# chacorp/latent-nerf-test

Measured on AMD Instinct MI355X. Metric: latent-frames/sec (64x64x4, 128^3 grid), render forward+backward, higher is better.
Workload: dtype bf16

## Files before the change

### latent-nerf-test_amd/csrc/grid_gather.hip

```cpp
#include "grid_shared.h"

namespace lnerf {

template <typename TT> struct CellRaw;
template <> struct CellRaw<uint16_t> {
    uint32_t d[8];
    __device__ __forceinline__ void load_pair(const uint16_t *lt, uint32_t row, int c) {
        const uint2 v = *reinterpret_cast<const uint2 *>(lt + (int64_t)row * 2);
        d[c] = v.x; d[c + 1] = v.y;
    }
    __device__ __forceinline__ void load_one(const uint16_t *lt, uint32_t row, int c) {
        d[c] = reinterpret_cast<const uint32_t *>(lt)[row];
    }
    __device__ __forceinline__ void load_quad(const uint16_t *lt, uint32_t r0, uint32_t r1, int c) {
        const uint4 v = *reinterpret_cast<const uint4 *>(lt + (int64_t)(r0 & ~3u) * 2);
        const uint32_t k0 = r0 & 3u, k1 = r1 & 3u;
        d[c] = (k0 & 2u) ? ((k0 & 1u) ? v.w : v.z) : ((k0 & 1u) ? v.y : v.x);
        d[c + 1] = (k1 & 2u) ? ((k1 & 1u) ? v.w : v.z) : ((k1 & 1u) ? v.y : v.x);
    }
    static constexpr bool kHasQuad = true;
    __device__ __forceinline__ void swap_pair(int c) { const uint32_t t = d[c]; d[c] = d[c + 1]; d[c + 1] = t; }
    __device__ __forceinline__ void zero() {
#pragma unroll
        for (int i = 0; i < 8; ++i) d[i] = 0u;
    }
    __device__ __forceinline__ void take_from_lane(int src) {
#pragma unroll
        for (int i = 0; i < 8; ++i) d[i] = (uint32_t)__builtin_amdgcn_ds_bpermute(src << 2, (int)d[i]);
    }
    __device__ __forceinline__ float2 get(int c) const {
        return make_float2(__uint_as_float(d[c] << 16), __uint_as_float(d[c] & 0xFFFF0000u));
    }
};
template <> struct CellRaw<float> {
    float2 d[8];
    __device__ __forceinline__ void load_pair(const float *lt, uint32_t row, int c) {
        const float4 v = *reinterpret_cast<const float4 *>(lt + (int64_t)row * 2);
        d[c] = make_float2(v.x, v.y); d[c + 1] = make_float2(v.z, v.w);
    }
    __device__ __forceinline__ void load_one(const float *lt, uint32_t row, int c) {
        d[c] = reinterpret_cast<const float2 *>(lt)[row];
    }
    __device__ __forceinline__ void load_quad(const float *, uint32_t, uint32_t, int) {}
    static constexpr bool kHasQuad = false;
    __device__ __forceinline__ void swap_pair(int c) { const float2 t = d[c]; d[c] = d[c + 1]; d[c + 1] = t; }
    __device__ __forceinline__ void zero() {
#pragma unroll
        for (int i = 0; i < 8; ++i) d[i] = make_float2(0.f, 0.f);
    }
    __device__ __forceinline__ void take_from_lane(int src) {
#pragma unroll
        for (int i = 0; i < 8; ++i) {
            d[i].x = __int_as_float(__builtin_amdgcn_ds_bpermute(src << 2, __float_as_int(d[i].x)));
            d[i].y = __int_as_float(__builtin_amdgcn_ds_bpermute(src << 2, __float_as_int(d[i].y)));
        }
    }
    __device__ __forceinline__ float2 get(int c) const { return d[c]; }
};

template <typename TT, typename TO>
__global__ void __launch_bounds__(256)
k_grid_forward(const float *__restrict__ xyzs, float bound, const TT *__restrict__ table, GridMeta meta, int64_t m_host,
               const int32_t *__restrict__ m_dev, int64_t level_stride, TO *__restrict__ feat, int pair_loads,
               int dedup_max_res) {
    int64_t M = m_host;
    if (m_dev) { const int64_t md = *m_dev; M = md < M ? md : M; }
    const TileMap tm = tile_map(0, meta.num_levels);
    const int l = tm.level;
    const float scale = meta.scales[l];
    const uint32_t res = (uint32_t)meta.res[l];
    const uint32_t off = (uint32_t)meta.offsets[l];
    const uint32_t hsize = (uint32_t)(meta.offsets[l + 1] - meta.offsets[l]);
    const TT *lt = table + (int64_t)off * 2;
    const bool dense = (uint64_t)(res + 1) * (res + 1) * (res + 1) <= (uint64_t)hsize;
    const bool pow2 = (hsize & (hsize - 1u)) == 0u;
    const bool dedup = (int)res <= dedup_max_res;
    const int lane = lane_id();
    for (int64_t tile = tm.tile0; tile * 256 < M; tile += tm.tstep) {
        const int64_t m = tile * 256 + threadIdx.x;
        const bool valid = m < M;
        LevelPos p;
        p.gx = p.gy = p.gz = 0u; p.fx = p.fy = p.fz = 0.f;
        if (valid) p = level_pos(xyzs, m, bound, scale);
        uint32_t rows[8];
        corner_rows(p.gx, p.gy, p.gz, res, hsize, rows, meta.blocked);
        bool fetch = valid;
        int src = lane;
        if (dedup) {
            const RunInfo ri = wave_cell_runs(p.gx, p.gy, p.gz, valid, lane);
            src = ri.start;
            fetch = valid && ri.start == lane;
        }
        CellRaw<TT> cell;
        cell.zero();
        if (fetch) {
            if (pair_loads && dense) {
#pragma unroll
                for (int c = 0; c < 8; c += 2) cell.load_pair(lt, rows[c], c);
            } else if (meta.blocked == 2) {
#pragma unroll
                for (int c = 0; c < 8; ++c) cell.load_one(lt, rows[c], c);
            } else if (pair_loads == 2 && CellRaw<TT>::kHasQuad && pow2 && (p.gx & 3u) != 3u) {
#pragma unroll
                for (int c = 0; c < 8; c += 2) cell.load_quad(lt, rows[c], rows[c + 1], c);
            } else if (pair_loads && pow2 && !(p.gx & 1u)) {
#pragma unroll
                for (int c = 0; c < 8; c += 2) {
                    cell.load_pair(lt, rows[c] & ~1u, c);
                    if (rows[c] & 1u) cell.swap_pair(c);
                }
            } else {
#pragma unroll
                for (int c = 0; c < 8; ++c) cell.load_one(lt, rows[c], c);
            }
        }
        if (dedup) cell.take_from_lane(src);
        float a0 = 0.f, a1 = 0.f;
#pragma unroll
        for (int c = 0; c < 8; ++c) {
            const uint32_t bx = c & 1, by = (c >> 1) & 1, bz = (c >> 2) & 1;
            const float wx = bx ? p.fx : 1.0f - p.fx;
            const float wy = by ? p.fy : 1.0f - p.fy;
            const float wz = bz ? p.fz : 1.0f - p.fz;
            const float w = (wx * wy) * wz;
            const float2 v = cell.get(c);
            a0 = fmaf(w, v.x, a0);
            a1 = fmaf(w, v.y, a1);
        }
        if (valid) Feat2<TO>::store(feat, (int64_t)l * level_stride + m, a0, a1);
    }
}

template <typename TG>
__global__ void __launch_bounds__(256)
k_grid_backward_atomic(const float *__restrict__ xyzs, float bound, const TG *__restrict__ dfeat, GridMeta meta,
                       int64_t m_host, const int32_t *__restrict__ m_dev, int64_t level_stride,
                       float *__restrict__ dtable, int variant) {
    int64_t M = m_host;
    if (m_dev) { const int64_t md = *m_dev; M = md < M ? md : M; }
    const TileMap tm = tile_map(variant, meta.num_levels);
    if (!tm.ok) return;
    const int l = tm.level;
    const float scale = meta.scales[l];
    const uint32_t res = (uint32_t)meta.res[l];
    const uint32_t off = (uint32_t)meta.offsets[l];
    const uint32_t hsize = (uint32_t)(meta.offsets[l + 1] - meta.offsets[l]);
    float *lt = dtable + (int64_t)off * 2;
    for (int64_t tile = tm.tile0; tile * 256 < M; tile += tm.tstep) {
        const int64_t m = tile * 256 + threadIdx.x;
        if (m >= M) continue;
        const LevelPos p = level_pos(xyzs, m, bound, scale);
        const float2 gg = Feat2<TG>::load(dfeat + ((int64_t)l * level_stride + m) * 2, 0);
        uint32_t rows[8];
        corner_rows(p.gx, p.gy, p.gz, res, hsize, rows, meta.blocked);
#pragma unroll
        for (int c = 0; c < 8; ++c) {
            const uint32_t bx = c & 1, by = (c >> 1) & 1, bz = (c >> 2) & 1;
            const uint32_t row = rows[c];
            const float wx = bx ? p.fx : 1.0f - p.fx;
            const float wy = by ? p.fy : 1.0f - p.fy;
            const float wz = bz ? p.fz : 1.0f - p.fz;
            const float w = (wx * wy) * wz;
            atomicAdd(lt + (int64_t)row * 2, w * gg.x);
            atomicAdd(lt + (int64_t)row * 2 + 1, w * gg.y);
        }
    }
}

static void launch_dims(int variant, int L, int64_t m_host, dim3 &grid) {
    const int64_t tiles = div_up(m_host, 256);
    if (variant == 0) {
        int64_t gx = tiles < 1 ? 1 : tiles;
        if (gx > 2048) gx = 2048;
        grid = dim3((unsigned)gx, (unsigned)L, 1);
    } else {
        const int lv_per_xcd = (L + 7) / 8;
        int64_t per_level = tiles < 1 ? 1 : tiles;
        if (per_level > 256) per_level = 256;
        grid = dim3((unsigned)(8 * lv_per_xcd * per_level), 1, 1);
    }
}

void launch_grid_backward_atomic(const float *xyzs, float bound, const float *dfeat, const GridMeta &meta, int64_t m_host,
                                 const int32_t *m_dev, int64_t level_stride, float *dtable, int variant, hipStream_t s) {
    dim3 grid;
    launch_dims(variant, meta.num_levels, m_host, grid);
    hipLaunchKernelGGL((k_grid_backward_atomic<float>), grid, dim3(256), 0, s, xyzs, bound, dfeat, meta, m_host, m_dev,
                       level_stride, dtable, variant);
}

}

using namespace lnerf;

extern "C" {

int lnerf_grid_encode_forward(const float *xyzs, float bound, const void *table, int table_dtype, int num_levels,
                              int level_dim, const int32_t *offsets_host, const float *scales_host,
                              const int32_t *res_host, int64_t m_host, const int32_t *m_dev, int64_t level_stride,
                              void *feat, int feat_dtype, int variant, lnerf_stream_t stream) {
    GridMeta meta;
    const int blocked = variant & (LNERF_GRID_BLOCKED | LNERF_GRID_TILED);
    variant &= ~(LNERF_GRID_BLOCKED | LNERF_GRID_TILED);
    int rc = fill_meta("grid_encode_forward", meta, num_levels, level_dim, offsets_host, scales_host, res_host, blocked);
    if (rc) return rc;
    LNERF_REQUIRE(m_host >= 0 && level_stride >= m_host, "grid_encode_forward: need 0 <= m_host <= level_stride");
    LNERF_REQUIRE(bound > 0.f, "grid_encode_forward: bound must be > 0");
    LNERF_REQUIRE(variant == 0, "grid_encode_forward: unknown variant %d", variant);
    LNERF_REQUIRE((table_dtype == LNERF_F32 || table_dtype == LNERF_BF16) &&
                      (feat_dtype == LNERF_F32 || feat_dtype == LNERF_BF16),
                  "grid_encode_forward: bad dtype tag");
    if (m_host == 0) return LNERF_OK;
    LNERF_REQUIRE(xyzs && table && feat, "grid_encode_forward: null pointer");
    dim3 grid;
    launch_dims(0, num_levels, m_host, grid);
    hipStream_t s = as_stream(stream);
#define LAUNCH_FWD(TT, TO)                                                                                         \
    hipLaunchKernelGGL((k_grid_forward<TT, TO>), grid, dim3(256), (size_t)g_gather_lds_pad, s, xyzs, bound, (const TT *)table, meta, m_host, \
                       m_dev, level_stride, (TO *)feat, g_gather_pairs, g_gather_dedup_res)
    if (table_dtype == LNERF_F32 && feat_dtype == LNERF_F32) LAUNCH_FWD(float, float);
    else if (table_dtype == LNERF_F32) LAUNCH_FWD(float, uint16_t);
    else if (feat_dtype == LNERF_F32) LAUNCH_FWD(uint16_t, float);
    else LAUNCH_FWD(uint16_t, uint16_t);
#undef LAUNCH_FWD
    LNERF_CHECK_LAUNCH("grid_encode_forward");
    return LNERF_OK;
}

}
```

Measured before the change: 2751.

## Specialize grid forward gather by span and prefetch next tile positions

Turns the runtime choice of gather path (dense pair, quad, pair, single loads) into template specializations, so each kernel instance carries one straight-line load path. The position of the next tile is loaded ahead of time, with sched barriers and asm register pins to overlap that load with the current gather. Row addresses are computed with 32-bit offsets, and a host check rejects levels larger than 4 GiB. The pins and prefetch add register pressure and can cut occupancy. The feature pointer offset now multiplies by 2, which may change indexing if Feat2 store already accounted for two channels.

```diff
diff --git a/latent-nerf-test_amd/csrc/grid_gather.hip b/latent-nerf-test_amd/csrc/grid_gather.hip
--- a/latent-nerf-test_amd/csrc/grid_gather.hip
+++ b/latent-nerf-test_amd/csrc/grid_gather.hip
@@ -1,28 +1,49 @@
 #include "grid_shared.h"
 
 namespace lnerf {
+
+typedef uint32_t u32x2 __attribute__((ext_vector_type(2)));
+typedef uint32_t u32x4 __attribute__((ext_vector_type(4)));
+
+template <typename TT> __device__ __forceinline__ const uint32_t *row_ptr(const TT *lt, uint32_t row) {
+    return reinterpret_cast<const uint32_t *>(reinterpret_cast<const char *>(lt) + (size_t)(row * (uint32_t)(2 * sizeof(TT))));
+}
 
 template <typename TT> struct CellRaw;
 template <> struct CellRaw<uint16_t> {
+    u32x4 a[4];
     uint32_t d[8];
-    __device__ __forceinline__ void load_pair(const uint16_t *lt, uint32_t row, int c) {
-        const uint2 v = *reinterpret_cast<const uint2 *>(lt + (int64_t)row * 2);
-        d[c] = v.x; d[c + 1] = v.y;
-    }
-    __device__ __forceinline__ void load_one(const uint16_t *lt, uint32_t row, int c) {
-        d[c] = reinterpret_cast<const uint32_t *>(lt)[row];
-    }
-    __device__ __forceinline__ void load_quad(const uint16_t *lt, uint32_t r0, uint32_t r1, int c) {
-        const uint4 v = *reinterpret_cast<const uint4 *>(lt + (int64_t)(r0 & ~3u) * 2);
-        const uint32_t k0 = r0 & 3u, k1 = r1 & 3u;
-        d[c] = (k0 & 2u) ? ((k0 & 1u) ? v.w : v.z) : ((k0 & 1u) ? v.y : v.x);
-        d[c + 1] = (k1 & 2u) ? ((k1 & 1u) ? v.w : v.z) : ((k1 & 1u) ? v.y : v.x);
-    }
-    static constexpr bool kHasQuad = true;
-    __device__ __forceinline__ void swap_pair(int c) { const uint32_t t = d[c]; d[c] = d[c + 1]; d[c + 1] = t; }
-    __device__ __forceinline__ void zero() {
-#pragma unroll
-        for (int i = 0; i < 8; ++i) d[i] = 0u;
+    static constexpr int kMaxSpan = 4;
+    static constexpr int kOwn = 8;
+    template <int SPAN> __device__ __forceinline__ void load_a(const uint16_t *lt, uint32_t row, int i) {
+        const uint32_t *p = row_ptr(lt, row);
+        if (SPAN == 4) {
+            a[i] = *reinterpret_cast<const u32x4 *>(p);
+        } else {
+            const u32x2 v = *reinterpret_cast<const u32x2 *>(p);
+            a[i].x = v.x; a[i].y = v.y;
+        }
+    }
+    __device__ __forceinline__ void load_own(const uint16_t *lt, uint32_t row, int c) { d[c] = *row_ptr(lt, row); }
+    __device__ __forceinline__ void open_raw() {
+        asm volatile("" : "=v"(a[0]), "=v"(a[1]), "=v"(a[2]), "=v"(a[3]), "=v"(d[0]), "=v"(d[1]), "=v"(d[2]), "=v"(d[3]),
+                          "=v"(d[4]), "=v"(d[5]), "=v"(d[6]), "=v"(d[7]));
+    }
+    __device__ __forceinline__ void pin_raw() {
+        asm volatile("" : "+v"(a[0]), "+v"(a[1]), "+v"(a[2]), "+v"(a[3]), "+v"(d[0]), "+v"(d[1]), "+v"(d[2]), "+v"(d[3]),
+                          "+v"(d[4]), "+v"(d[5]), "+v"(d[6]), "+v"(d[7]));
+    }
+    template <int SPAN> static __device__ __forceinline__ uint32_t pick(const u32x4 &v, uint32_t k) {
+        if (SPAN == 2) return (k & 1u) ? v.y : v.x;
+        return (k & 2u) ? ((k & 1u) ? v.w : v.z) : ((k & 1u) ? v.y : v.x);
+    }
+    template <int SPAN, bool DENSE> __device__ __forceinline__ void take_pairs(const uint32_t rows[8], bool own) {
+        if (SPAN == 1 || own) return;
+#pragma unroll
+        for (int i = 0; i < 4; ++i) {
+            d[2 * i] = DENSE ? a[i].x : pick<SPAN>(a[i], rows[2 * i]);
+            d[2 * i + 1] = DENSE ? a[i].y : pick<SPAN>(a[i], rows[2 * i + 1]);
+        }
     }
     __device__ __forceinline__ void take_from_lane(int src) {
 #pragma unroll
@@ -33,57 +54,75 @@
     }
 };
 template <> struct CellRaw<float> {
-    float2 d[8];
-    __device__ __forceinline__ void load_pair(const float *lt, uint32_t row, int c) {
-        const float4 v = *reinterpret_cast<const float4 *>(lt + (int64_t)row * 2);
-        d[c] = make_float2(v.x, v.y); d[c + 1] = make_float2(v.z, v.w);
-    }
-    __device__ __forceinline__ void load_one(const float *lt, uint32_t row, int c) {
-        d[c] = reinterpret_cast<const float2 *>(lt)[row];
-    }
-    __device__ __forceinline__ void load_quad(const float *, uint32_t, uint32_t, int) {}
-    static constexpr bool kHasQuad = false;
-    __device__ __forceinline__ void swap_pair(int c) { const float2 t = d[c]; d[c] = d[c + 1]; d[c + 1] = t; }
-    __device__ __forceinline__ void zero() {
-#pragma unroll
-        for (int i = 0; i < 8; ++i) d[i] = make_float2(0.f, 0.f);
+    u32x4 a[4];
+    u32x2 d[8];
+    static constexpr int kMaxSpan = 2;
+    static constexpr int kOwn = 4;
+    template <int SPAN> __device__ __forceinline__ void load_a(const float *lt, uint32_t row, int i) {
+        const uint32_t *p = row_ptr(lt, row);
+        if (SPAN == 2) {
+            a[i] = *reinterpret_cast<const u32x4 *>(p);
+        } else {
+            const u32x2 v = *reinterpret_cast<const u32x2 *>(p);
+            a[i].x = v.x; a[i].y = v.y;
+        }
+    }
+    __device__ __forceinline__ void load_own(const float *lt, uint32_t row, int c) {
+        d[c] = *reinterpret_cast<const u32x2 *>(row_ptr(lt, row));
+    }
+    __device__ __forceinline__ void open_raw() {
+        asm volatile("" : "=v"(a[0]), "=v"(a[1]), "=v"(a[2]), "=v"(a[3]), "=v"(d[1]), "=v"(d[3]), "=v"(d[5]), "=v"(d[7]));
+    }
+    __device__ __forceinline__ void pin_raw() {
+        asm volatile("" : "+v"(a[0]), "+v"(a[1]), "+v"(a[2]), "+v"(a[3]), "+v"(d[1]), "+v"(d[3]), "+v"(d[5]), "+v"(d[7]));
+    }
+    static __device__ __forceinline__ u32x2 pick(const u32x4 &v, uint32_t k) {
+        return (k & 1u) ? u32x2{v.z, v.w} : u32x2{v.x, v.y};
+    }
+    template <int SPAN, bool DENSE> __device__ __forceinline__ void take_pairs(const uint32_t rows[8], bool own) {
+#pragma unroll
+        for (int i = 0; i < 4; ++i) d[2 * i] = (SPAN == 1 || DENSE) ? u32x2{a[i].x, a[i].y} : pick(a[i], rows[2 * i]);
+        if (SPAN == 1 || own) return;
+#pragma unroll
+        for (int i = 0; i < 4; ++i) d[2 * i + 1] = DENSE ? u32x2{a[i].z, a[i].w} : pick(a[i], rows[2 * i + 1]);
     }
     __device__ __forceinline__ void take_from_lane(int src) {
 #pragma unroll
         for (int i = 0; i < 8; ++i) {
-            d[i].x = __int_as_float(__builtin_amdgcn_ds_bpermute(src << 2, __float_as_int(d[i].x)));
-            d[i].y = __int_as_float(__builtin_amdgcn_ds_bpermute(src << 2, __float_as_int(d[i].y)));
-        }
-    }
-    __device__ __forceinline__ float2 get(int c) const { return d[c]; }
+            d[i].x = (uint32_t)__builtin_amdgcn_ds_bpermute(src << 2, (int)d[i].x);
+            d[i].y = (uint32_t)__builtin_amdgcn_ds_bpermute(src << 2, (int)d[i].y);
+        }
+    }
+    __device__ __forceinline__ float2 get(int c) const { return make_float2(__uint_as_float(d[c].x), __uint_as_float(d[c].y)); }
 };
 
-template <typename TT, typename TO>
-__global__ void __launch_bounds__(256)
-k_grid_forward(const float *__restrict__ xyzs, float bound, const TT *__restrict__ table, GridMeta meta, int64_t m_host,
-               const int32_t *__restrict__ m_dev, int64_t level_stride, TO *__restrict__ feat, int pair_loads,
-               int dedup_max_res) {
-    int64_t M = m_host;
-    if (m_dev) { const int64_t md = *m_dev; M = md < M ? md : M; }
-    const TileMap tm = tile_map(0, meta.num_levels);
-    const int l = tm.level;
-    const float scale = meta.scales[l];
-    const uint32_t res = (uint32_t)meta.res[l];
-    const uint32_t off = (uint32_t)meta.offsets[l];
-    const uint32_t hsize = (uint32_t)(meta.offsets[l + 1] - meta.offsets[l]);
-    const TT *lt = table + (int64_t)off * 2;
-    const bool dense = (uint64_t)(res + 1) * (res + 1) * (res + 1) <= (uint64_t)hsize;
-    const bool pow2 = (hsize & (hsize - 1u)) == 0u;
-    const bool dedup = (int)res <= dedup_max_res;
+struct PosRaw {
+    float x, y, z;
+    __device__ __forceinline__ void request(const float *__restrict__ xyzs, int64_t m, int64_t M) {
+        m = m < M ? m : M - 1;
+        x = xyzs[m * 3]; y = xyzs[m * 3 + 1]; z = xyzs[m * 3 + 2];
+    }
+    __device__ __forceinline__ void pin() { asm volatile("" : "+v"(x), "+v"(y), "+v"(z)); }
+};
+
+template <typename TT, typename TO, int SPAN, bool DENSE>
+__device__ __forceinline__ void gather_tiles(const float *__restrict__ xyzs, float bound, const TT *__restrict__ lt,
+                                             float scale, uint32_t res, uint32_t hsize, int layout, bool dedup, int64_t M,
+                                             const TileMap &tm, TO *__restrict__ lfeat) {
+    constexpr uint32_t kmask = DENSE ? 0u : (uint32_t)(SPAN - 1);
     const int lane = lane_id();
+    PosRaw pos;
+    pos.request(xyzs, tm.tile0 * 256 + threadIdx.x, M);
+    pos.pin();
     for (int64_t tile = tm.tile0; tile * 256 < M; tile += tm.tstep) {
         const int64_t m = tile * 256 + threadIdx.x;
         const bool valid = m < M;
-        LevelPos p;
-        p.gx = p.gy = p.gz = 0u; p.fx = p.fy = p.fz = 0.f;
-        if (valid) p = level_pos(xyzs, m, bound, scale);
+        PosRaw next;
+        next.request(xyzs, m + tm.tstep * 256 < M ? m + tm.tstep * 256 : m, M);
+        __builtin_amdgcn_sched_barrier(0);
+        const LevelPos p = level_pos_xyz(pos.x, pos.y, pos.z, bound, scale);
         uint32_t rows[8];
-        corner_rows(p.gx, p.gy, p.gz, res, hsize, rows, meta.blocked);
+        corner_rows(p.gx, p.gy, p.gz, res, hsize, rows, layout);
         bool fetch = valid;
         int src = lane;
         if (dedup) {
@@ -91,29 +130,21 @@
             src = ri.start;
             fetch = valid && ri.start == lane;
         }
+        const bool own = SPAN == 1 || (!DENSE && (p.gx & (uint32_t)(SPAN - 1)) == (uint32_t)(SPAN - 1));
         CellRaw<TT> cell;
-        cell.zero();
+        cell.open_raw();
         if (fetch) {
-            if (pair_loads && dense) {
-#pragma unroll
-                for (int c = 0; c < 8; c += 2) cell.load_pair(lt, rows[c], c);
-            } else if (meta.blocked == 2) {
-#pragma unroll
-                for (int c = 0; c < 8; ++c) cell.load_one(lt, rows[c], c);
-            } else if (pair_loads == 2 && CellRaw<TT>::kHasQuad && pow2 && (p.gx & 3u) != 3u) {
-#pragma unroll
-                for (int c = 0; c < 8; c += 2) cell.load_quad(lt, rows[c], rows[c + 1], c);
-            } else if (pair_loads && pow2 && !(p.gx & 1u)) {
-#pragma unroll
-                for (int c = 0; c < 8; c += 2) {
-                    cell.load_pair(lt, rows[c] & ~1u, c);
-                    if (rows[c] & 1u) cell.swap_pair(c);
-                }
-            } else {
-#pragma unroll
-                for (int c = 0; c < 8; ++c) cell.load_one(lt, rows[c], c);
+            if (CellRaw<TT>::kOwn == 4 || (SPAN > 1 && !own)) {
+#pragma unroll
+                for (int i = 0; i < 4; ++i) cell.template load_a<SPAN>(lt, rows[2 * i] & ~kmask, i);
             }
-        }
+            if (own) {
+#pragma unroll
+                for (int c = (CellRaw<TT>::kOwn == 4 ? 1 : 0); c < 8; c += 8 / CellRaw<TT>::kOwn) cell.load_own(lt, rows[c], c);
+            }
+        }
+        cell.pin_raw();
+        cell.template take_pairs<SPAN, DENSE>(rows, own);
         if (dedup) cell.take_from_lane(src);
         float a0 = 0.f, a1 = 0.f;
 #pragma unroll
@@ -127,8 +158,45 @@
             a0 = fmaf(w, v.x, a0);
             a1 = fmaf(w, v.y, a1);
         }
-        if (valid) Feat2<TO>::store(feat, (int64_t)l * level_stride + m, a0, a1);
-    }
+        next.pin();
+        if (valid) Feat2<TO>::store(lfeat, m, a0, a1);
+        pos = next;
+    }
+}
+
+template <typename TT, typename TO>
+__global__ void __launch_bounds__(256)
+k_grid_forward(const float *__restrict__ xyzs, float bound, const TT *__restrict__ table, GridMeta meta, int64_t m_host,
+               const int32_t *__restrict__ m_dev, int64_t level_stride, TO *__restrict__ feat, int pair_loads,
+               int dedup_max_res) {
+    int64_t M = m_host;
+    if (m_dev) { const int64_t md = *m_dev; M = md < M ? md : M; }
+    const TileMap tm = tile_map(0, meta.num_levels);
+    if (tm.tile0 * 256 >= M) return;
+    const int l = tm.level;
+    const float scale = meta.scales[l];
+    const uint32_t res = (uint32_t)meta.res[l];
+    const uint32_t off = (uint32_t)meta.offsets[l];
+    const uint32_t hsize = (uint32_t)(meta.offsets[l + 1] - meta.offsets[l]);
+    const TT *lt = table + (int64_t)off * 2;
+    TO *lfeat = feat + (int64_t)l * level_stride * 2;
+    const bool dense = (uint64_t)(res + 1) * (res + 1) * (res + 1) <= (uint64_t)hsize;
+    const bool pow2 = (hsize & (hsize - 1u)) == 0u;
+    const bool dedup = (int)res <= dedup_max_res;
+#define GATHER_TILES(SPAN, DENSE) \
+    gather_tiles<TT, TO, SPAN, DENSE>(xyzs, bound, lt, scale, res, hsize, meta.blocked, dedup, M, tm, lfeat)
+    if (pair_loads && dense) {
+        GATHER_TILES(2, true);
+    } else if (pair_loads && pow2 && meta.blocked != 2 && !dense && hsize >= 4u) {
+        if (pair_loads == 2 && CellRaw<TT>::kMaxSpan == 4) {
+            if constexpr (CellRaw<TT>::kMaxSpan == 4) GATHER_TILES(4, false);
+        } else {
+            GATHER_TILES(2, false);
+        }
+    } else {
+        GATHER_TILES(1, false);
+    }
+#undef GATHER_TILES
 }
 
 template <typename TG>
@@ -212,6 +280,9 @@
                   "grid_encode_forward: bad dtype tag");
     if (m_host == 0) return LNERF_OK;
     LNERF_REQUIRE(xyzs && table && feat, "grid_encode_forward: null pointer");
+    for (int l = 0; l < num_levels; ++l)
+        LNERF_REQUIRE((uint64_t)(offsets_host[l + 1] - offsets_host[l]) * (table_dtype == LNERF_F32 ? 8u : 4u) <= (1ull << 32),
+                      "grid_encode_forward: level %d is larger than 4 GiB", l);
     dim3 grid;
     launch_dims(0, num_levels, m_host, grid);
     hipStream_t s = as_stream(stream);
```

Result: no change. 2764, median of 6 (+0.5%).
